# mathdiane/dNMF

Measured on AMD Instinct MI355X. Metric: frames/sec demixed, 512x512xT K=100, higher is better.
Workload: dtype f32

## Files before the change

### dnmf_amd/_lib.py

```python
from __future__ import annotations

import ctypes as C
import os

_HERE = os.path.dirname(os.path.abspath(__file__))
LIB_PATH = os.environ.get("DNMF_LIB") or os.path.join(_HERE, "libdnmf_hip.so")
ABI_VERSION = 6

_vp, _i, _l, _sz, _d = C.c_void_p, C.c_int, C.c_long, C.c_size_t, C.c_double

SIGNATURES = {
    "dnmf_version": (_i, []),
    "dnmf_last_error": (C.c_char_p, []),
    "dnmf_build_stamp": (C.c_char_p, []),
    "dnmf_padded_k": (_i, [_i]),
    "dnmf_pack_footprints": (_i, [_vp, _l, _i, _vp, _i, _vp]),
    "dnmf_warp_gather": (_i, [_vp, _i, _i, _i, _i, _vp, _i, _vp, _i, _vp, _vp, _vp]),
    "dnmf_halo_voxels": (_l, [_i, _i, _i]),
    "dnmf_halo_row": (_i, [_i, _i]),
    "dnmf_recon_image": (_i, [_vp, _i, _i, _i, _i, _i, _vp, _l, _vp, _i, _vp, _l, _vp]),
    "dnmf_warp_recon_grad_workspace": (_sz, [_i, _i, _i, _i]),
    "dnmf_warp_recon_grad": (_i, [_vp, _l, _vp, _vp, _l, _vp, _vp, _i, _i, _i, _vp, _i, _vp, _i, _i, _vp, _vp, _vp,
                                  _vp, _vp, _vp, _sz, _vp]),
    "dnmf_warp_gram_rhs_workspace": (_sz, [_l, _i, _i]),
    "dnmf_warp_gram_rhs": (_i, [_vp, _i, _i, _l, _i, _i, _i, _vp, _i, _vp, _i, _vp, _l, _vp, _vp, _vp, _vp, _sz,
                                _vp]),
    "dnmf_warp_gram_rhs_bf16": (_i, [_vp, _i, _i, _l, _i, _i, _i, _vp, _i, _vp, _i, _vp, _l, _vp, _vp, _vp, _vp, _sz,
                                     _vp]),
    "dnmf_sparse_k": (_i, [_i]),
    "dnmf_pack_footprints_sparse": (_i, [_vp, _l, _i, _vp, _vp, _i, _vp, _vp]),
    "dnmf_warp_gram_rhs_sparse_workspace": (_sz, [_l, _i, _i]),
    "dnmf_warp_gram_rhs_sparse": (_i, [_vp, _i, _i, _vp, _vp, _i, _i, _i, _vp, _i, _vp, _i, _vp, _l, _vp, _vp, _vp, _vp,
                                       _sz, _vp, _vp]),
    "dnmf_warp_gram_rhs_sparse_lt_workspace": (_sz, [_l, _i, _i]),
    "dnmf_warp_gram_rhs_sparse_lt": (_i, [_vp, _i, _i, _vp, _vp, _i, _i, _i, _vp, _i, _vp, _i, _vp, _l, _vp, _vp, _vp, _vp,
                                          _sz, _vp, _vp]),
    "dnmf_mu_temporal": (_i, [_vp, _vp, _vp, _l, _i, _i, _i, _vp]),
    "dnmf_mu_temporal_nbr": (_i, [_vp, _vp, _vp, _l, _i, _i, _i, _vp, _i, _vp]),
    "dnmf_mu_temporal_slots": (_i, [_vp, _i, _i, _vp, _vp, _l, _i, _i, _i, _vp, _i, _vp]),
    "dnmf_warp_gram_rhs_lists_chunks": (_i, [_i, _i, _i, _i]),
    "dnmf_mu_temporal_step": (_i, [_vp, _vp, _vp, _vp, _l, _i, _i, _d, _vp, _vp, _vp]),
    "dnmf_hals_temporal": (_i, [_vp, _vp, _vp, _l, _i, _i, _i, _vp, _i, _vp, _vp]),
    "dnmf_hals_temporal_slots": (_i, [_vp, _i, _i, _vp, _vp, _l, _i, _i, _i, _vp, _i, _vp, _vp]),
    "dnmf_hals_temporal_step": (_i, [_vp, _vp, _vp, _l, _i, _i, _d, _i, _vp, _i, _vp]),
    "dnmf_hals_temporal_kkt": (_i, [_vp, _vp, _vp, _l, _i, _i, _d, _vp, _i, _vp, _vp]),
    "dnmf_spatial_accum": (_i, [_vp, _l, _vp, _vp, _l, _vp, _l, _vp, _i, _l, _i, _vp, _vp, _i, _vp]),
    "dnmf_mu_spatial": (_i, [_vp, _vp, _vp, _vp, _d, _l, _i, _vp]),
    "dnmf_image_iwarp_workspace": (_sz, [_i, _i, _i, _i]),
    "dnmf_image_iwarp": (_i, [_vp, _l, _vp, _i, _i, _i, _vp, _i, _vp, _i, _vp, _l, _vp, _sz, _i, _vp, _vp]),
    "dnmf_image_iwarp_channels": (_i, [_vp, _l, _l, _i, _vp, _i, _i, _i, _vp, _i, _vp, _i, _vp, _l, _l, _vp, _sz, _i, _vp,
                                        _vp]),
    "dnmf_adam_epoch_workspace": (_sz, [_i]),
    "dnmf_adam_epoch": (_i, [_vp, _vp, _vp, _vp, _i, _l, _vp, _vp, _i, _d, _d, _d, _d, _i, _vp, _sz, _vp]),
    "dnmf_render_frames": (_i, [_vp, _vp, _i, _i, _i, _i, _i, _i, _i, _d, _d, _vp, _l, _vp]),
    "dnmf_lists_axis_masks_bytes": (_sz, [_i, _i, _i, _i]),
    "dnmf_pack_footprints_lists": (_i, [_vp, _i, _i, _i, _i, _vp, _vp, _vp, _vp, _vp, _vp]),
    "dnmf_warp_gram_rhs_lists_workspace": (_sz, [_i, _i, _i, _i, _i, _i]),
    "dnmf_warp_gram_rhs_lists": (_i, [_vp, _vp, _vp, _vp, _i, _i, _i, _i, _i, _vp, _i, _vp, _i, _vp, _l, _vp, _vp, _vp,
                                      _vp, _sz, _vp, _vp]),
    "dnmf_recon_image_lists": (_i, [_vp, _vp, _i, _i, _i, _i, _vp, _l, _vp, _i, _vp, _l, _vp]),
    "dnmf_recon_image_lists_ex": (_i, [_vp, _vp, _i, _i, _i, _i, _vp, _l, _vp, _i, _vp, _l, _i, _vp]),
    "dnmf_motion_grad_lists_workspace": (_sz, [_i, _i, _i, _i, _i]),
    "dnmf_motion_grad_lists": (_i, [_vp, _vp, _i, _vp, _l, _vp, _l, _vp, _i, _i, _i, _vp, _i, _vp, _i, _i, _vp, _vp, _vp, _i,
                                    _vp, _sz, _vp]),
    "dnmf_spatial_lists_tiles": (_l, [_i, _i, _i]),
    "dnmf_spatial_lists_setup": (_i, [_vp, _i, _i, _i, _i, _vp, _vp]),
    "dnmf_spatial_accum_lists_workspace": (_sz, [_i, _i, _i, _l, _i]),
    "dnmf_spatial_accum_lists": (_i, [_vp, _l, _vp, _vp, _l, _vp, _i, _i, _i, _i, _i, _vp, _l, _vp, _vp, _vp, _sz, _vp]),
    "dnmf_spatial_accum_lists_channels": (_i, [_vp, _l, _l, _i, _vp, _vp, _vp, _l, _vp, _i, _i, _i, _i, _i, _vp, _l, _vp, _vp,
                                                _vp, _sz, _vp]),
    "dnmf_mu_spatial_lists": (_i, [_vp, _vp, _vp, _vp, _vp, _d, _i, _i, _i, _i, _vp, _vp]),
    "dnmf_register_patches_grid": (_i, [_i, _i, _i, _vp, _vp, _vp, _vp]),
    "dnmf_register_patches_workspace": (_sz, [_i, _i, _i, _vp, _vp, _i]),
    "dnmf_register_patches": (_i, [_vp, _l, _vp, _i, _vp, _i, _i, _i, _vp, _vp, _vp, _i, _i, C.c_float, _vp, _vp, _vp, _sz, _vp]),
    "dnmf_rigid_correct_workspace": (_sz, [_i, _i, _i, _i]),
    "dnmf_rigid_correct": (_i, [_vp, _l, _vp, _i, _vp, _i, _i, _i, _vp, _i, C.c_float, _i, _vp, _vp, _l, _vp, _vp, _vp, _sz, _vp]),
    "dnmf_apply_pwrigid_workspace": (_sz, [_i, _i, _i, _vp, _vp, _i]),
    "dnmf_apply_pwrigid": (_i, [_vp, _l, _vp, _i, _i, _i, _i, _vp, _vp, _vp, C.c_float, _vp, _l, _vp, _vp, _vp, _sz, _vp]),
    "dnmf_apply_shifts_points": (_i, [_vp, _i, _vp, _i, _i, _vp, _vp, _vp]),
    "dnmf_nearest_points_workspace": (_sz, [_i, _i]),
    "dnmf_nearest_points": (_i, [_vp, _i, _l, _i, _vp, _l, _i, _i, _vp, _l, _vp, _l, _vp, _l, _vp, _sz, _vp]),
    "dnmf_fit_quadratic_warp": (_i, [_vp, _i, _i, _i, _vp, _i, _i, _i, _i, _d, _vp, _vp, _vp]),
    "dnmf_invert_quadratic_warp": (_i, [_vp, _i, _vp, _i, _vp, _i, _vp, _d, _vp, _vp]),
    "dnmf_roi_signals": (_i, [_vp, _l, _i, _i, _i, _vp, _i, _i, _i, _vp, _vp, _vp]),
    "dnmf_detect_neurons_workspace": (_sz, [_vp, _i, _d]),
    "dnmf_detect_neurons": (_i, [_vp, _vp, _i, _d, _d, _d, _d, _vp, _vp, _vp, _vp, _sz, _vp]),
    "dnmf_track_neurons": (_i, [_vp, _l, _vp, _i, _vp, _vp, _i, _i, _i, _d, _vp, _d, _vp, _vp, _vp, _vp, _vp]),
    "dnmf_warp_normal_eqs_workspace": (_sz, [_i, _i, _i, _i]),
    "dnmf_warp_normal_eqs": (_i, [_vp, _l, _vp, _vp, _l, _vp, _i, _i, _i, _vp, _i, _vp, _i, _vp, _vp, _vp, _i, _vp, _sz, _vp]),
    "dnmf_lm_step": (_i, [_vp, _vp, _vp, _i, _i, _vp, _vp, _i, _vp, _vp, _vp, _vp, _vp, _vp, _vp, _vp, _d, _d, _d, _d, _i, _vp]),
    "dnmf_lm_step_smooth": (_i, [_vp, _vp, _vp, _i, _i, _vp, _vp, _vp, _i, _vp, _vp, _vp, _vp, _vp, _vp, _vp, _vp, _d, _d, _d,
                                 _d, _i, _vp, _d, _vp, _vp]),
    "dnmf_warp_pullback": (_i, [_vp, _l, _l, _i, _vp, _i, _i, _i, _vp, _i, _vp, _i, _vp, _l, _l, _i, C.c_float, _vp, _vp, _vp]),
# ... 56 lines not shown
```

### dnmf_amd/csrc/warp_gram_lists.hip

```cpp
#include <cstdlib>

#include "warp_gram_lists.hpp"

namespace dnmf {

__global__ __launch_bounds__(256) void lists_axis_masks_kernel(const int *__restrict__ bbox, int K, Volume vol, int NW,
                                                               unsigned long long *__restrict__ masks) {
    const long e = (long)blockIdx.x * 256 + threadIdx.x;
    if (e >= axis_masks_entries(vol)) return;
    const int S[3] = {vol.X, vol.Y, vol.Z};
    long o = e;
    int d = 0;
    while (o >= 2L * (S[d] + 2)) o -= 2L * (S[d] + 2), ++d;
    const bool hi_table = o >= S[d] + 2;
    const int i = hi_table ? (int)(o - (S[d] + 2)) : (int)o - 1;
    for (int w = 0; w < NW; ++w) {
        unsigned long long m = 0;
        for (int j = 0; j < 64; ++j) {
            const int k = 64 * w + j;
            if (k >= K) break;
            const int lo = bbox[k * 6 + 2 * d], hi = bbox[k * 6 + 2 * d + 1];
            const bool in = lo <= hi && (hi_table ? hi >= i : lo <= i);
            m |= (unsigned long long)in << j;
        }
        masks[e * NW + w] = m;
    }
}

template <int NW>
__global__ __launch_bounds__(256) void lists_tilemask_kernel(ListParams p) {
    const long id = (long)blockIdx.x * 256 + threadIdx.x;
    if (id >= (long)p.B * p.ntiles) return;
    const int b = (int)(id / p.ntiles), q = (int)(id - (long)b * p.ntiles);
    const Volume vol = p.vol;
    const int t = p.times ? p.times[b] : b;
    float bt[30];
    load_beta(p.beta, p.T, t, bt);
    const int qx = q % p.ntx, rest = q / p.ntx, qz = rest % p.ntz, qy = rest / p.ntz;
    const int tx = LISTS_VPL << p.lgx, ty = 1 << p.lgy, tz = 1 << p.lgz;
    const int S[3] = {vol.X, vol.Y, vol.Z};
    const int first[3] = {qx * tx, qy * ty, qz * tz}, size[3] = {tx, ty, tz};
    float lo[3], hi[3];
#pragma unroll
    for (int d = 0; d < 3; ++d) lo[d] = (float)first[d], hi[d] = (float)min(first[d] + size[d] - 1, S[d] - 1);
    const bool hasz = vol.Z > 1;
    unsigned long long m[NW];
#pragma unroll
    for (int w = 0; w < NW; ++w) m[w] = ~0ull;
    int ta[3] = {0, 0, 0}, tc[3] = {0, 0, 0};
    bool finite = true;
#pragma unroll
    for (int d = 0; d < 3; ++d) {
        int a = 0, c = 0;
        if ((d < 2 || hasz) && !tap_range(bt, vol, d, lo, hi, hasz, a, c)) {
#pragma unroll
            for (int w = 0; w < NW; ++w) m[w] = 0;
            finite = false;
            continue;
        }
        ta[d] = a, tc[d] = c;
        const unsigned long long *LO = p.axis_masks + (axis_masks_offset(vol, d, 0) + (min(c, S[d]) + 1 < 0 ? 0 : min(c, S[d]) + 1)) * NW;
        const unsigned long long *HI = p.axis_masks + (axis_masks_offset(vol, d, 1) + min(max(a, 0), S[d] + 1)) * NW;
#pragma unroll
        for (int w = 0; w < NW; ++w) m[w] &= LO[w] & HI[w];
    }
#pragma unroll
    for (int w = 0; w < NW; ++w) p.tile_masks[id * NW + w] = m[w];
    int2 reg = make_int2(-1, 0);
    if (vol.Z <= 2 && finite && p.hl.Xp >= LISTS_RR && p.hl.rowf >= LISTS_RC && p.hl.Xp < 32768 && p.hl.rowf < 65536) {
        const int ax = max(ta[0], -HALO), cx = min(tc[0], vol.X + 1), ay = max(ta[1], -HALO), cy = min(tc[1], vol.Y + 1);
        const int r0 = min(ax + HALO, p.hl.Xp - LISTS_RR), c0 = min(((ay + HALO) * vol.Z) & ~3, p.hl.rowf - LISTS_RC);
        if (cx >= ax && cy >= ay && cx + HALO - r0 < LISTS_RR && (cy + HALO) * vol.Z + vol.Z - 1 - c0 < LISTS_RC)
            reg = make_int2(r0, c0);
    }
    int nlist = 0;
    unsigned ids = 0xffffffffu;
#pragma unroll
    for (int w = 0; w < NW; ++w) {
        unsigned long long rem = m[w];
        while (rem) {
            if (nlist < 4) ids = (ids & ~(0xffu << (8 * nlist))) | ((unsigned)(64 * w + __builtin_ctzll(rem)) << (8 * nlist));
            ++nlist, rem &= rem - 1;
        }
    }
    const int place = (qx < 65536 && rest < 32768) ? (qx | rest << 16) : -1;
    p.tile_desc[id] = make_int4(reg.x < 0 ? -1 : (reg.x << 16 | reg.y), (int)ids, nlist, place);
}

__global__ __launch_bounds__(256) void gram_lists_finish_kernel(const float *__restrict__ slab, int nchunks, int nslot,
                                                                const int *__restrict__ pair_slot, int K,
                                                                float *__restrict__ G, float *__restrict__ r) {
    const int b = blockIdx.x;
    const float *src = slab + (long)b * nchunks * nslot;
    for (int e = threadIdx.x; e < K * K + K; e += blockDim.x) {
        const int slot = e < K * K ? pair_slot[e] : e - K * K;
        float s = 0.0f;
        if (slot != nslot - 1)
            for (int c = 0; c < nchunks; ++c) s += src[(long)c * nslot + slot];
        if (e < K * K)
            G[(long)b * K * K + e] = s;
        else
            r[(long)b * K + (e - K * K)] = s;
    }
}

__global__ void lists_init_kernel(int *bbox, int K) {
    const int i = blockIdx.x * blockDim.x + threadIdx.x;
    if (i < K * 6) bbox[i] = (i & 1) ? -1 : 0x7fffffff;
}

__global__ __launch_bounds__(256) void lists_transpose_kernel(const float *__restrict__ A, long P, int K, Volume vol,
                                                              HaloLayout hl, float *__restrict__ At,
                                                              int *__restrict__ bbox) {
    __shared__ float tile[32][33];
    const long p0 = (long)blockIdx.x * 32;
    const int k0 = blockIdx.y * 32;
    const int tx = threadIdx.x & 31, ty = threadIdx.x >> 5;
    for (int i = ty; i < 32; i += 8) {
        const long pp = p0 + i;
        const int k = k0 + tx;
        tile[i][tx] = (pp < P && k < K) ? A[pp * K + k] : 0.0f;
    }
    __syncthreads();
    for (int i = ty; i < 32; i += 8) {
        const int k = k0 + i;
        const long pp = p0 + tx;
        const bool in = k < K && pp < P;
        const float v = in ? tile[tx][i] : 0.0f;
        int x = 0, y = 0, z = 0;
        if (in) {
            voxel_xyz(pp, vol, x, y, z);
            At[(long)k * hl.Pp + (long)(x + HALO) * hl.rowf + (long)(y + HALO) * vol.Z + z] = v;
        }
        const bool nz = v != 0.0f;
        const unsigned long long any = __ballot(nz);
        if (any == 0) continue;
        int lo[3] = {nz ? x : 0x7fffffff, nz ? y : 0x7fffffff, nz ? z : 0x7fffffff};
        int hi[3] = {nz ? x : -1, nz ? y : -1, nz ? z : -1};
#pragma unroll
// ... 46 lines not shown
        for (int l = k + 1; l < K; ++l) {
            const int v = meets(k, l) ? s++ : trash;
            pair_slot[k * K + l] = v;
            pair_slot[l * K + k] = v;
        }
    }
}

static void lists_tile_shape(const Volume &vol, int &lgx, int &lgy, int &lgz, int &ntx, int &nty, int &ntz, int &ntiles) {
    lgz = vol.Z == 1 ? 0 : (vol.Z == 2 ? 1 : 2);
    lgy = vol.Z == 1 ? 5 : 4;
    lgx = 6 - lgy - lgz;
    const int tx = LISTS_VPL << lgx, ty = 1 << lgy, tz = 1 << lgz;
    ntx = (vol.X + tx - 1) / tx;
    ntz = (vol.Z + tz - 1) / tz;
    nty = (vol.Y + ty - 1) / ty;
    ntiles = ntx * nty * ntz;
}

static long lists_max_chunks(int B) {
    const long want = (LISTS_ITEMS + B - 1) / B;
    return want < 1 ? 1 : (want > 64 ? 64 : want);
}

static void lists_choose_chunks(int ntiles, int B, int &nchunks, int &chunk_len) {
    long want = lists_max_chunks(B);
    if (const char *e = getenv("DNMF_LISTS_CHUNKS")) {
        const long n = strtol(e, nullptr, 10);
        if (n >= 1 && n <= want) want = n;
    }
    if (want > ntiles) want = ntiles;
    chunk_len = (int)((ntiles + want - 1) / want);
    nchunks = (ntiles + chunk_len - 1) / chunk_len;
}

static int lists_words(int K) { return K <= 64 ? 1 : (K <= 128 ? 2 : 4); }

static int lists_passes(int chunk_len) {
    if (const char *e = getenv("DNMF_LISTS_PASSES")) {
        if (e[0] == '1' && e[1] == 0) return 1;
        if (e[0] == '2' && e[1] == 0) return 2;
    }
    return chunk_len < 100 ? 1 : 2;
}

static void lists_plan(ListParams &p) {
    lists_tile_shape(p.vol, p.lgx, p.lgy, p.lgz, p.ntx, p.nty, p.ntz, p.ntiles);
    lists_choose_chunks(p.ntiles, p.B, p.nchunks, p.chunk_len);
    p.tables = p.nchunks * lists_passes(p.chunk_len);
}

template <int NW>
static void launch_tilemask(const ListParams &p, hipStream_t st) {
    const long nthreads = (long)p.B * p.ntiles;
    hipLaunchKernelGGL((lists_tilemask_kernel<NW>), dim3((unsigned)((nthreads + 255) / 256)), dim3(256), 0, st, p);
}

SideStream &side_stream() {
    static SideStream per_device[64];
    static std::mutex create;
    int dev = 0;
    if (hipGetDevice(&dev) != hipSuccess || dev < 0 || dev >= 64) dev = 0;
    SideStream &ss = per_device[dev];
    std::lock_guard<std::mutex> hold(create);
    if (!ss.stream) {
        hipStream_t s = nullptr;
        hipEvent_t a = nullptr, b = nullptr;
        if (hipStreamCreateWithFlags(&s, hipStreamNonBlocking) == hipSuccess &&
            hipEventCreateWithFlags(&a, hipEventDisableTiming) == hipSuccess &&
            hipEventCreateWithFlags(&b, hipEventDisableTiming) == hipSuccess)
            ss.stream = s, ss.fork = a, ss.join = b;
    }
    return ss;
}

}

extern "C" {

size_t dnmf_lists_axis_masks_bytes(int X, int Y, int Z, int K) {
    if (X <= 0 || Y <= 0 || Z <= 0 || K <= 0 || K > 64 * dnmf::LISTS_MAXW) return 0;
    return (size_t)dnmf::axis_masks_entries(dnmf::make_volume(X, Y, Z)) * dnmf::lists_words(K) * sizeof(unsigned long long);
}

int dnmf_pack_footprints_lists(const float *A, int X, int Y, int Z, int K, float *At, int *bbox, int *pair_slot,
                               int *nslot, void *axis_masks, dnmf_stream_t stream) {
    using namespace dnmf;
    DNMF_REQUIRE(A && At && bbox && pair_slot && nslot && axis_masks, DNMF_E_NULL, "dnmf_pack_footprints_lists: NULL buffer");
    DNMF_REQUIRE(X > 0 && Y > 0 && Z > 0 && K > 0, DNMF_E_SHAPE, "dnmf_pack_footprints_lists: X=%d Y=%d Z=%d K=%d", X, Y, Z,
                 K);
    DNMF_REQUIRE(K <= 64 * LISTS_MAXW, DNMF_E_UNSUPPORTED, "dnmf_pack_footprints_lists: K=%d > %d", K, 64 * LISTS_MAXW);
    const Volume vol = make_volume(X, Y, Z);
    const HaloLayout hl = make_halo_layout(X, Y, Z);
    hipStream_t st = (hipStream_t)stream;
    hipError_t e = hipMemsetAsync(At, 0, (size_t)K * hl.Pp * sizeof(float), st);
    DNMF_REQUIRE(e == hipSuccess, (int)e, "dnmf_pack_footprints_lists: hipMemsetAsync: %s", hipGetErrorString(e));
    hipLaunchKernelGGL(lists_init_kernel, dim3((K * 6 + 255) / 256), dim3(256), 0, st, bbox, K);
    hipLaunchKernelGGL(lists_transpose_kernel, dim3((unsigned)((vol.P + 31) / 32), (unsigned)((K + 31) / 32)), dim3(256), 0,
                       st, A, vol.P, K, vol, hl, At, bbox);
    hipLaunchKernelGGL(lists_pairs_kernel, dim3(1), dim3(256), 0, st, bbox, K, pair_slot, nslot);
    hipLaunchKernelGGL(lists_axis_masks_kernel, dim3((unsigned)((axis_masks_entries(vol) + 255) / 256)), dim3(256), 0, st, bbox,
                       K, vol, lists_words(K), static_cast<unsigned long long *>(axis_masks));
    return check_launch("dnmf_pack_footprints_lists");
}

static size_t lists_slab_bytes(int nslot, int B) {
    const size_t tables = 2 * (size_t)dnmf::lists_max_chunks(B);
    return ((size_t)B * tables * (size_t)nslot * sizeof(float) + 255) / 256 * 256;
}

static size_t lists_masks_bytes(int K, int B, int ntiles) {
    return ((size_t)B * ntiles * dnmf::lists_words(K) * sizeof(unsigned long long) + 15) / 16 * 16;
}

size_t dnmf_warp_gram_rhs_lists_workspace(int nslot, int K, int X, int Y, int Z, int B) {
    using namespace dnmf;
    if (nslot <= 0 || B <= 0 || K <= 0 || K > 64 * LISTS_MAXW || X <= 0 || Y <= 0 || Z <= 0) return 0;
    int lgx, lgy, lgz, ntx, nty, ntz, ntiles;
    lists_tile_shape(make_volume(X, Y, Z), lgx, lgy, lgz, ntx, nty, ntz, ntiles);
    return lists_slab_bytes(nslot, B) + lists_masks_bytes(K, B, ntiles) + (size_t)B * ntiles * sizeof(int4);
}

int dnmf_warp_gram_rhs_lists(const float *At, const int *bbox, const int *pair_slot, const void *axis_masks, int nslot, int K,
                             int X, int Y, int Z, const float *beta, int T, const int *times, int B, const float *frames,
                             long ldf, const int *frame_ids, float *G, float *r, void *workspace, size_t workspace_bytes,
                             unsigned long long *counters, dnmf_stream_t stream) {
    using namespace dnmf;
    DNMF_REQUIRE(At && bbox && pair_slot && axis_masks && beta && frames && workspace && (!G == !r), DNMF_E_NULL,
                 "dnmf_warp_gram_rhs_lists: NULL buffer");
    DNMF_REQUIRE(X > 0 && Y > 0 && Z > 0 && K > 0 && T > 0 && B > 0 && nslot > K, DNMF_E_SHAPE,
                 "dnmf_warp_gram_rhs_lists: X=%d Y=%d Z=%d K=%d T=%d B=%d nslot=%d", X, Y, Z, K, T, B, nslot);
    DNMF_REQUIRE(K <= 64 * LISTS_MAXW, DNMF_E_UNSUPPORTED, "dnmf_warp_gram_rhs_lists: K=%d > %d", K, 64 * LISTS_MAXW);
    DNMF_REQUIRE(nslot <= LISTS_MAX_SLOTS, DNMF_E_UNSUPPORTED,
                 "dnmf_warp_gram_rhs_lists: %d pattern slots > %d (footprints overlap too much for this kernel)", nslot,
                 LISTS_MAX_SLOTS);
    ListParams p;
    p.vol = make_volume(X, Y, Z);
    p.hl = make_halo_layout(X, Y, Z);
    DNMF_REQUIRE(ldf >= p.vol.P, DNMF_E_SHAPE, "dnmf_warp_gram_rhs_lists: ldf=%ld < P=%ld", ldf, p.vol.P);
    DNMF_REQUIRE(p.hl.Pp < (1L << 29) && p.hl.row4 < (1 << 23) && p.hl.Xp < (1 << 23), DNMF_E_UNSUPPORTED,
                 "dnmf_warp_gram_rhs_lists: volume %dx%dx%d too large for 32-bit tap offsets", X, Y, Z);
    p.At = At, p.bbox = bbox, p.pair_slot = pair_slot, p.nslot = nslot, p.K = K;
    p.axis_masks = static_cast<const unsigned long long *>(axis_masks);
    p.beta = beta, p.T = T, p.times = times, p.B = B;
    p.frames = frames, p.ldf = ldf, p.frame_ids = frame_ids;
    p.slab = static_cast<float *>(workspace);
    p.tile_masks = reinterpret_cast<unsigned long long *>(static_cast<char *>(workspace) + lists_slab_bytes(nslot, B));
    p.counters = counters;
    lists_plan(p);
    DNMF_REQUIRE(workspace_bytes >= dnmf_warp_gram_rhs_lists_workspace(nslot, K, X, Y, Z, B), DNMF_E_WORKSPACE,
                 "dnmf_warp_gram_rhs_lists: workspace %zu < %zu bytes", workspace_bytes,
                 dnmf_warp_gram_rhs_lists_workspace(nslot, K, X, Y, Z, B));
    hipStream_t st = (hipStream_t)stream;
    const long nitems = (long)p.nchunks * B;
    const unsigned nwg = (unsigned)((nitems + 3) / 4);
    const int nw = lists_words(K);
    p.tile_desc = reinterpret_cast<int4 *>(reinterpret_cast<char *>(p.tile_masks) + lists_masks_bytes(K, B, p.ntiles));
    const size_t lds = (((size_t)4 * nslot + 3) & ~(size_t)3) * sizeof(float) +
                       (Z <= 2 ? (size_t)4 * LISTS_NG * LISTS_REGION * sizeof(float) : 0);
    if (nw == 1) launch_tilemask<1>(p, st);
    else if (nw == 2) launch_tilemask<2>(p, st);
    else launch_tilemask<4>(p, st);
    if (Z > 1) {
        launch_lists_z(p, nwg, lds, st, nw);
    } else {
        if (nw == 1) launch_lists_t<1, 1>(p, nwg, lds, st);
        else if (nw == 2) launch_lists_t<1, 2>(p, nwg, lds, st);
        else launch_lists_t<1, 4>(p, nwg, lds, st);
    }
    if (G)
        hipLaunchKernelGGL(gram_lists_finish_kernel, dim3((unsigned)B), dim3(256), 0, st, p.slab, p.tables, nslot,
                           pair_slot, K, G, r);
    return check_launch("dnmf_warp_gram_rhs_lists");
}

int dnmf_warp_gram_rhs_lists_chunks(int X, int Y, int Z, int B) {
    using namespace dnmf;
    if (X <= 0 || Y <= 0 || Z <= 0 || B <= 0) return 0;
    ListParams p{};
    p.vol = make_volume(X, Y, Z), p.B = B;
    lists_plan(p);
    return p.tables;
}

}
```

### dnmf_amd/csrc/warp_gram_lists.hpp

```cpp
#pragma once
#include <mutex>
#include <type_traits>

#include "warp_taps.hpp"

namespace dnmf {

typedef float f32x4 __attribute__((ext_vector_type(4)));


constexpr int LISTS_WAVES = 4;
constexpr int LISTS_WAVES_Z2 = 4;
constexpr int LISTS_WAVES_Z2L = 3;
constexpr int LISTS_WAVES_Z3 = 3;

constexpr int LISTS_NG = 4;
constexpr int LISTS_LGV = 2;
constexpr int LISTS_VPL = 1 << LISTS_LGV;
constexpr int LISTS_MAXW = 4;
constexpr long LISTS_ITEMS = 16384;
constexpr int LISTS_MAX_SLOTS = 3800;
constexpr int LISTS_RR = 12, LISTS_RC = 40;
constexpr int LISTS_REGION = LISTS_RR * LISTS_RC;
static_assert(LISTS_RC % 4 == 0 && LISTS_REGION / 4 <= 128 && LISTS_REGION / 4 > 64, "stage_dma moves two pieces per lane");

struct ListParams {
    const float *At;
    const int *bbox;
    const int *pair_slot;
    const unsigned long long *axis_masks;
    int nslot;
    int K;
    Volume vol;
    HaloLayout hl;
    const float *beta;
    int T;
    const int *times;
    int B;
    const float *frames;
    long ldf;
    const int *frame_ids;
    float *slab;
    unsigned long long *tile_masks;
    int4 *tile_desc;
    int nchunks, chunk_len;
    int tables;
    int lgx, lgy, lgz;
    int ntx, nty, ntz, ntiles;
    unsigned long long *counters;
};

__host__ __device__ inline long axis_masks_offset(const Volume &vol, int d, int hi_table) {
    const int S[3] = {vol.X, vol.Y, vol.Z};
    long o = 0;
    for (int e = 0; e < d; ++e) o += 2L * (S[e] + 2);
    return o + (hi_table ? S[d] + 2 : 0);
}
__host__ __device__ inline long axis_masks_entries(const Volume &vol) { return 2L * (vol.X + vol.Y + vol.Z + 6); }

template <int ZM, int NW, int FAST, bool F32OFF, int PASS>
__global__ __launch_bounds__(256, (ZM == 1 ? LISTS_WAVES : (ZM == 2 ? (PASS == 2 ? LISTS_WAVES_Z2L : LISTS_WAVES_Z2) : LISTS_WAVES_Z3))) void warp_gram_lists_kernel(ListParams p) {
    constexpr bool LONGPASS = PASS == 2;
    extern __shared__ float s_tab[];
    constexpr bool HASZ = ZM > 1;
    constexpr int NPAIR = LISTS_NG * (LISTS_NG + 1) / 2;
    const int lane = threadIdx.x & 63;
    const int wave = __builtin_amdgcn_readfirstlane(threadIdx.x >> 6);
    const long item = (long)blockIdx.x * 4 + wave;
    if (item >= (long)p.nchunks * p.B) return;
    const int chunk = (int)(item / p.B);
    const int b = (int)(item - (long)chunk * p.B);
    const int t = p.times ? p.times[b] : b;
    const float *__restrict__ yb = p.frames + (long)(p.frame_ids ? p.frame_ids[b] : b) * p.ldf;
    const Volume vol = p.vol;
    const HaloLayout hl = p.hl;
    const int K = p.K;
    const size_t plane = (size_t)hl.Pp * 4u;

    float bt[30];
    load_beta(p.beta, p.T, t, bt);

    float *tab = s_tab + (size_t)wave * p.nslot;
    for (int i = lane; i < p.nslot; i += 64) tab[i] = 0.0f;
    const unsigned tab_lds = (unsigned)(size_t)(__attribute__((address_space(3))) float *)tab;
    char *stage_lds = reinterpret_cast<char *>(s_tab + (((size_t)4 * p.nslot + 3) & ~(size_t)3)) +
                      (size_t)wave * (LISTS_NG * LISTS_REGION * 4);
    constexpr int PPR = LISTS_RC / 4;
    const int piece_row[2] = {lane / PPR, (lane + 64) / PPR};
    const int piece_c4[2] = {lane - piece_row[0] * PPR, lane + 64 - piece_row[1] * PPR};
    const int4 *__restrict__ descs = p.tile_desc + (long)b * p.ntiles;

    const int lgx = p.lgx, lgz = p.lgz;
    const int lgy = p.lgy;
    const int lz = lane & ((1 << lgz) - 1), ly = (lane >> lgz) & ((1 << lgy) - 1), lx = lane >> (lgz + lgy);
    const int q_begin = chunk * p.chunk_len;
    const int q_end = min(q_begin + p.chunk_len, p.ntiles);
    const unsigned long long *__restrict__ masks = p.tile_masks + (long)b * p.ntiles * NW;
    unsigned long long n_eval = 0, n_pair = 0;
#ifdef DNMF_K3N_STAMPS
    unsigned long long st_acc[10] = {0, 0, 0, 0, 0, 0, 0, 0, 0, 0}, st_last = __builtin_amdgcn_s_memtime();
#define DNMF_STAMP(i)                                                     \
    {                                                                     \
        const unsigned long long now_ = __builtin_amdgcn_s_memtime();      \
        st_acc[i] += now_ - st_last, st_last = now_;                      \
    }
#else
#define DNMF_STAMP(i)
#endif

    __builtin_amdgcn_fence(__ATOMIC_RELEASE, "wavefront");
    __builtin_amdgcn_wave_barrier();
    __builtin_amdgcn_fence(__ATOMIC_ACQUIRE, "wavefront");

    auto add_slot = [&](int slot, float total_in_last_lane) {
        const unsigned addr = tab_lds + 4u * (unsigned)slot;
        if (lane == 63) asm volatile("ds_add_f32 %0, %1" : : "v"(addr), "v"(total_in_last_lane) : "memory");
    };
    auto pair_slot_of = [&](int k, int l) {
        return __builtin_amdgcn_readfirstlane(p.pair_slot[max(k, 0) * K + max(l, 0)]);
    };
    auto take_ids = [&](unsigned long long (&rem)[NW], int (&ks)[LISTS_NG]) {
#pragma unroll
        for (int i = 0; i < LISTS_NG; ++i) {
            int k = -1;
// ... 6 lines not shown
                found = found || take;
            }
            ks[i] = k;
        }
    };

    float acc_r[LISTS_NG], acc_p[NPAIR];
    int run_k[LISTS_NG];
    int run_n = 0;
    auto flush = [&]() {
        if (run_n == 0) return;
        auto go = [&](auto nn) {
            constexpr int N = decltype(nn)::value;
            int sl[N][N];
#pragma unroll
            for (int i = 0; i < N; ++i)
#pragma unroll
                for (int j = i; j < N; ++j) sl[i][j] = pair_slot_of(run_k[i], run_k[j]);
            float sr[N], sp[N][N];
            int e = 0;
#pragma unroll
            for (int i = 0; i < N; ++i) {
                sr[i] = wave_sum_last(acc_r[i]);
#pragma unroll
                for (int j = i; j < N; ++j) sp[i][j] = wave_sum_last(acc_p[e++]);
            }
#pragma unroll
            for (int i = 0; i < N; ++i) {
                add_slot(run_k[i], sr[i]);
#pragma unroll
                for (int j = i; j < N; ++j) add_slot(sl[i][j], sp[i][j]);
            }
        };
        using std::integral_constant;
        switch (run_n) {
            case 1: go(integral_constant<int, 1>{}); break;
            case 2: go(integral_constant<int, 2>{}); break;
            case 3: go(integral_constant<int, 3>{}); break;
            default: go(integral_constant<int, 4>{}); break;
        }
        static_assert(LISTS_NG == 4, "the dispatch above lists the group sizes");
        run_n = 0;
    };

    float b2[30];
    double_beta(bt, b2);
    Monomials<HASZ> mono = monomials<HASZ>(0.0f, 0.0f, 0.0f);
    int row_of_c = -1;
    unsigned long long prev[NW];
#pragma unroll
    for (int wd = 0; wd < NW; ++wd) prev[wd] = 0;
    int prev_ids = -1;

    for (int q0 = q_begin; q0 < q_end; q0 += 64) {
      unsigned my_lo[NW], my_hi[NW];
      int my_reg = -1;
      int my_ids = -1, my_n = 0;
      int my_place = -1;
      {
          const int ql = min(q0 + lane, q_end - 1);
          if (PASS != 1) {
#pragma unroll
              for (int wd = 0; wd < NW; ++wd) {
                  const unsigned long long m = masks[(long)ql * NW + wd];
                  my_lo[wd] = (unsigned)m, my_hi[wd] = (unsigned)(m >> 32);
              }
          }
          const int4 dsc = descs[ql];
          my_reg = ZM == 3 ? -1 : dsc.x, my_ids = dsc.y, my_n = dsc.z, my_place = dsc.w;
      }
      if (LONGPASS) {
          int myn = 0;
#pragma unroll
          for (int wd = 0; wd < NW; ++wd) myn += __builtin_popcount(my_lo[wd]) + __builtin_popcount(my_hi[wd]);
          if (__ballot(myn > LISTS_NG) == 0) continue;
      }
      const int q1 = min(q0 + 64, q_end);
      for (int q = q0; q < q1; ++q) {
        const int jl = q - q0;
        unsigned long long msk[NW];
        int n = 0;
        bool same = true;
        int ids = -1;
        if (PASS == 1) {
            n = __builtin_amdgcn_readlane(my_n, jl);
            if (n == 0 || n > LISTS_NG) continue;
            ids = __builtin_amdgcn_readlane(my_ids, jl);
            same = ids == prev_ids;
            prev_ids = ids;
        } else {
#pragma unroll
            for (int wd = 0; wd < NW; ++wd) {
                msk[wd] = ((unsigned long long)(unsigned)__builtin_amdgcn_readlane((int)my_hi[wd], jl) << 32) |
                          (unsigned)__builtin_amdgcn_readlane((int)my_lo[wd], jl);
                n += __builtin_popcountll(msk[wd]);
                same = same && msk[wd] == prev[wd];
            }
        }
        if (n == 0 || (PASS == 1 && n > LISTS_NG) || (PASS == 2 && n <= LISTS_NG)) continue;
        DNMF_STAMP(0)
#ifdef DNMF_K3N_STAMPS
        st_acc[7] += 1, st_acc[8] += n > LISTS_NG, st_acc[9] += (!same || n > LISTS_NG) && run_n != 0;
#endif
        if (!same || n > LISTS_NG) flush();
        DNMF_STAMP(1)
        if (PASS != 1) {
#pragma unroll
            for (int wd = 0; wd < NW; ++wd) prev[wd] = n > LISTS_NG ? 0 : msk[wd];
        }

        const int place = __builtin_amdgcn_readlane(my_place, jl);
        const int qx = place >= 0 ? (place & 0xffff) : q % p.ntx, rest = place >= 0 ? (place >> 16) : q / p.ntx;
        if (rest != row_of_c) {
            const int qz = HASZ ? rest % p.ntz : 0, qy = HASZ ? rest / p.ntz : rest;
            mono = monomials<HASZ>(0.0f, (float)((qy << lgy) + ly), (float)((qz << lgz) + lz));
            row_of_c = rest;
        }
        const int qz = HASZ ? rest % p.ntz : 0, qy = HASZ ? rest / p.ntz : rest;
        const int y = (qy << lgy) + ly, z = (qz << lgz) + lz;
        const bool yz_in = y < vol.Y && z < vol.Z;
        int reg_r0 = -1, reg_c0 = 0;
        if (ZM != 3) {
            const int rg = __builtin_amdgcn_readlane(my_reg, jl);
            reg_r0 = rg < 0 ? -1 : rg >> 16, reg_c0 = rg & 0xffff;
        }
        const bool staged = ZM != 3 && reg_r0 >= 0 && n <= (PASS == 2 ? 2 : 1) * LISTS_NG;
        const float lds_origin = 4.0f * (float)((HALO - reg_r0) * LISTS_RC + HALO * (ZM == 2 ? 2 : 1) - reg_c0);
        const unsigned reg_goff = (unsigned)(reg_r0 * hl.row4 + reg_c0 * 4);

        auto stage_load = [&](int k, f32x4 (&piece)[2]) {
            const char *__restrict__ Ak = reinterpret_cast<const char *>(p.At) + (size_t)k * plane + reg_goff;
#pragma unroll
            for (int j = 0; j < 2; ++j) {
                unsigned o = (unsigned)(piece_row[j] * hl.row4 + piece_c4[j] * 16);
                asm("" : "+v"(o));
                piece[j] = (j == 0 || lane + 64 < LISTS_REGION / 4) ? *reinterpret_cast<const f32x4 *>(Ak + o)
                                                                   : f32x4{0.f, 0.f, 0.f, 0.f};
            }
// ... 268 lines not shown
            }
            DNMF_STAMP(6)
            continue;
        }
        unsigned long long rem1[NW];
#pragma unroll
        for (int wd = 0; wd < NW; ++wd) rem1[wd] = msk[wd];
        for (int g1 = 0; g1 < n; g1 += LISTS_NG) {
            int kA[LISTS_NG];
            float aA[LISTS_NG][LISTS_VPL];
            take_ids(rem1, kA);
#pragma unroll
            for (int i = 0; i < LISTS_NG; ++i)
                if (kA[i] >= 0) {
                    eval(kA[i], aA[i]);
                } else {
#pragma unroll
                    for (int v = 0; v < LISTS_VPL; ++v) aA[i][v] = 0.0f;
                }
#pragma unroll
            for (int i = 0; i < LISTS_NG; ++i) {
                if (kA[i] < 0) continue;
                add_slot(kA[i], wave_sum_last(dot4(aA[i], yv, 0.0f)));
#pragma unroll
                for (int j = i; j < LISTS_NG; ++j)
                    if (kA[j] >= 0) add_slot(pair_slot_of(kA[i], kA[j]), wave_sum_last(dot4(aA[i], aA[j], 0.0f)));
            }
            unsigned long long rem2[NW];
#pragma unroll
            for (int wd = 0; wd < NW; ++wd) rem2[wd] = rem1[wd];
            for (int g2 = g1 + LISTS_NG; g2 < n; g2 += LISTS_NG) {
                int kB[LISTS_NG];
                take_ids(rem2, kB);
#pragma unroll
                for (int j = 0; j < LISTS_NG; ++j) {
                    if (kB[j] < 0) continue;
                    float aB[LISTS_VPL];
                    eval(kB[j], aB);
                    int sl[LISTS_NG];
#pragma unroll
                    for (int i = 0; i < LISTS_NG; ++i) sl[i] = pair_slot_of(kA[i], kB[j]);
                    float sp[LISTS_NG];
#pragma unroll
                    for (int i = 0; i < LISTS_NG; ++i) sp[i] = wave_sum_last(dot4(aA[i], aB, 0.0f));
#pragma unroll
                    for (int i = 0; i < LISTS_NG; ++i)
                        if (kA[i] >= 0) add_slot(sl[i], sp[i]);
                }
            }
        }
        DNMF_STAMP(6)
        }
      }
    }
    flush();

    __builtin_amdgcn_fence(__ATOMIC_RELEASE, "wavefront");
    __builtin_amdgcn_wave_barrier();
    __builtin_amdgcn_fence(__ATOMIC_ACQUIRE, "wavefront");
    float *out = p.slab + ((long)b * p.tables + (LONGPASS ? p.nchunks : 0) + chunk) * p.nslot;
    for (int i = lane; i < p.nslot; i += 64) out[i] = tab[i];
    if (p.counters && lane == 0) {
        atomicAdd(&p.counters[0], n_eval);
        atomicAdd(&p.counters[1], n_pair);
#ifdef DNMF_K3N_STAMPS
        DNMF_STAMP(5)
        for (int i = 0; i < 10; ++i) atomicAdd(&p.counters[2 + i], st_acc[i]);
#endif
    }
}
#undef DNMF_STAMP

struct SideStream {
    std::mutex lock;
    hipStream_t stream = nullptr;
    hipEvent_t fork = nullptr, join = nullptr;
};
SideStream &side_stream();

template <int ZM, int NW, int FAST, bool F32OFF>
void launch_lists_passes(const ListParams &p, unsigned nwg, size_t lds, hipStream_t st) {
    if (p.tables == p.nchunks) {
        hipLaunchKernelGGL((warp_gram_lists_kernel<ZM, NW, FAST, F32OFF, 0>), dim3(nwg), dim3(256), lds, st, p);
        return;
    }
    SideStream &ss = side_stream();
    std::lock_guard<std::mutex> hold(ss.lock);
    const bool forked = ss.stream && hipEventRecord(ss.fork, st) == hipSuccess &&
                        hipStreamWaitEvent(ss.stream, ss.fork, 0) == hipSuccess;
    if (forked) {
        hipLaunchKernelGGL((warp_gram_lists_kernel<ZM, NW, FAST, F32OFF, 2>), dim3(nwg), dim3(256), lds, ss.stream, p);
        const bool recorded = hipEventRecord(ss.join, ss.stream) == hipSuccess;
        hipLaunchKernelGGL((warp_gram_lists_kernel<ZM, NW, FAST, F32OFF, 1>), dim3(nwg), dim3(256), lds, st, p);
        if (!recorded || hipStreamWaitEvent(st, ss.join, 0) != hipSuccess)
            (void)hipStreamSynchronize(ss.stream);
    } else {
        hipLaunchKernelGGL((warp_gram_lists_kernel<ZM, NW, FAST, F32OFF, 1>), dim3(nwg), dim3(256), lds, st, p);
        hipLaunchKernelGGL((warp_gram_lists_kernel<ZM, NW, FAST, F32OFF, 2>), dim3(nwg), dim3(256), lds, st, p);
    }
}

template <int ZM, int NW>
void launch_lists_t(const ListParams &p, unsigned nwg, size_t lds, hipStream_t st) {
    if (p.vol.fastdiv && p.hl.f32off)
        launch_lists_passes<ZM, NW, 1, true>(p, nwg, lds, st);
    else if (p.vol.fastdiv)
// ... 9 lines not shown
```

### include/dnmf_hip.h

```cpp
#ifndef DNMF_HIP_H
#define DNMF_HIP_H

#include <stddef.h>

#ifdef __cplusplus
extern "C" {
#endif

#define DNMF_ABI_VERSION 6

#define DNMF_OK 0
#define DNMF_E_NULL (-1)
#define DNMF_E_SHAPE (-2)
#define DNMF_E_UNSUPPORTED (-3)
#define DNMF_E_WORKSPACE (-4)

typedef void *dnmf_stream_t;

#define DNMF_HALO 2
int dnmf_halo_row(int Y, int Z);
long dnmf_halo_voxels(int X, int Y, int Z);

int dnmf_version(void);
const char *dnmf_last_error(void);
const char *dnmf_build_stamp(void);

int dnmf_padded_k(int K);
int dnmf_pack_footprints(const float *A, long P, int K, float *Apk, int Kp, dnmf_stream_t stream);

int dnmf_warp_gather(const float *A, int X, int Y, int Z, int K, const float *beta, int T,
                     const int *times, int B, float *A_t, float *grid, dnmf_stream_t stream);

int dnmf_recon_image(const float *Apk, int X, int Y, int Z, int K, int Kp, const float *C, long ldc, const int *times,
                     int B, float *S, long lds, dnmf_stream_t stream);

size_t dnmf_warp_recon_grad_workspace(int X, int Y, int Z, int B);
int dnmf_warp_recon_grad(const float *S, long lds, const int *s_ids, const float *frames, long ldf,
                         const int *frame_ids, const float *gout, int X, int Y, int Z, const float *beta,
                         int T, const int *times, int B, int norm_frames, float *recon, float *grad, float *loss,
                         float *frame_loss, float *reg, void *workspace, size_t workspace_bytes,
                         dnmf_stream_t stream);

size_t dnmf_warp_gram_rhs_workspace(long P, int K, int B);
int dnmf_warp_gram_rhs(const float *Apk, int Kp, int K, long a_frame_stride, int X, int Y, int Z,
                       const float *beta, int T, const int *times, int B, const float *frames, long ldf,
                       const int *frame_ids, float *G, float *r, void *workspace, size_t workspace_bytes,
                       dnmf_stream_t stream);

int dnmf_warp_gram_rhs_bf16(const float *Apk, int Kp, int K, long a_frame_stride, int X, int Y, int Z,
                            const float *beta, int T, const int *times, int B, const float *frames, long ldf,
                            const int *frame_ids, float *G, float *r, void *workspace, size_t workspace_bytes,
                            dnmf_stream_t stream);

int dnmf_sparse_k(int K);
int dnmf_pack_footprints_sparse(const float *A, long P, int K, const int *order, float *Aps, int Ks,
                                unsigned char *row_mask, dnmf_stream_t stream);
size_t dnmf_warp_gram_rhs_sparse_workspace(long P, int K, int B);
int dnmf_warp_gram_rhs_sparse(const float *Aps, int Ks, int K, const int *order, const unsigned char *row_mask,
                              int X, int Y, int Z, const float *beta, int T, const int *times, int B,
                              const float *frames, long ldf, const int *frame_ids, float *G, float *r,
                              void *workspace, size_t workspace_bytes, unsigned long long *counters,
                              dnmf_stream_t stream);

size_t dnmf_warp_gram_rhs_sparse_lt_workspace(long P, int K, int B);
int dnmf_warp_gram_rhs_sparse_lt(const float *Aps, int Ks, int K, const int *order, const unsigned char *row_mask,
                                 int X, int Y, int Z, const float *beta, int T, const int *times, int B,
                                 const float *frames, long ldf, const int *frame_ids, float *G, float *r,
                                 void *workspace, size_t workspace_bytes, unsigned long long *counters,
                                 dnmf_stream_t stream);

size_t dnmf_lists_axis_masks_bytes(int X, int Y, int Z, int K);
int dnmf_pack_footprints_lists(const float *A, int X, int Y, int Z, int K, float *At, int *bbox, int *pair_slot,
                               int *nslot, void *axis_masks, dnmf_stream_t stream);
size_t dnmf_warp_gram_rhs_lists_workspace(int nslot, int K, int X, int Y, int Z, int B);
int dnmf_warp_gram_rhs_lists_chunks(int X, int Y, int Z, int B);
int dnmf_warp_gram_rhs_lists(const float *At, const int *bbox, const int *pair_slot, const void *axis_masks, int nslot,
                             int K, int X, int Y, int Z, const float *beta, int T, const int *times, int B,
                             const float *frames, long ldf, const int *frame_ids, float *G, float *r, void *workspace,
                             size_t workspace_bytes, unsigned long long *counters, dnmf_stream_t stream);

int dnmf_recon_image_lists(const float *At, const int *bbox, int K, int X, int Y, int Z, const float *C, long ldc,
                           const int *times, int B, float *S, long lds, dnmf_stream_t stream);
int dnmf_recon_image_lists_ex(const float *At, const int *bbox, int K, int X, int Y, int Z, const float *C, long ldc,
                              const int *times, int B, float *S, long lds, int skip_empty, dnmf_stream_t stream);

size_t dnmf_motion_grad_lists_workspace(int X, int Y, int Z, int chunk, int B);
int dnmf_motion_grad_lists(const float *At, const int *bbox, int K, const float *C, long ldc, const float *frames, long ldf,
                           const int *frame_ids, int X, int Y, int Z, const float *beta, int T, const int *times, int B,
                           int norm_frames, float *grad, float *frame_loss, float *reg, int chunk, void *workspace,
                           size_t workspace_bytes, dnmf_stream_t stream);

int dnmf_mu_temporal(const float *G, const float *r, float *C, long ldc, int K, int T, int iters,
                     dnmf_stream_t stream);
int dnmf_mu_temporal_nbr(const float *G, const float *r, float *C, long ldc, int K, int T, int iters, const int *nbr,
                         int NN, dnmf_stream_t stream);
int dnmf_mu_temporal_slots(const float *slab, int nchunks, int nslot, const int *pair_slot, float *C, long ldc, int K,
                           int T, int iters, const int *nbr, int NN, dnmf_stream_t stream);
int dnmf_mu_temporal_step(const float *G, const float *r, const double *Cin, double *Cout, long ldc, int K,
                          int T, double gamma, const double *c_left, const double *c_right,
                          dnmf_stream_t stream);

int dnmf_hals_temporal(const float *G, const float *r, float *C, long ldc, int K, int T, int iters, const int *nbr, int NN,
                       double *kkt, dnmf_stream_t stream);
int dnmf_hals_temporal_slots(const float *slab, int nchunks, int nslot, const int *pair_slot, float *C, long ldc, int K,
                             int T, int iters, const int *nbr, int NN, double *kkt, dnmf_stream_t stream);
int dnmf_hals_temporal_step(const float *G, const float *r, double *C, long ldc, int K, int T, double gamma, int parity,
                            const int *nbr, int NN, dnmf_stream_t stream);
int dnmf_hals_temporal_kkt(const float *G, const float *r, const double *C, long ldc, int K, int T, double gamma,
                           const int *nbr, int NN, double *kkt, dnmf_stream_t stream);

int dnmf_spatial_accum(const float *Y, long ldy, const int *frame_ids, const float *C, long ldc, const float *Ct,
                       long ldct, const int *times, int T, long P, int K, float *A1, float *Cs, int accumulate,
                       dnmf_stream_t stream);
int dnmf_mu_spatial(float *A, const float *A1, const float *Cs, const float *D, double gamma, long P, int K,
                    dnmf_stream_t stream);

#define DNMF_COMM_ID_BYTES 128
typedef void *dnmf_comm_t;
int dnmf_comm_unique_id(void *id_host);
int dnmf_comm_init(dnmf_comm_t *comm, const void *id_host, int nranks, int rank);
int dnmf_allreduce_sum_f32(dnmf_comm_t comm, float *buf, size_t count, dnmf_stream_t stream);
int dnmf_comm_destroy(dnmf_comm_t comm);

size_t dnmf_image_iwarp_workspace(int X, int Y, int Z, int B);
int dnmf_image_iwarp(const float *frames, long ldf, const int *frame_ids, int X, int Y, int Z, const float *beta,
                     int T, const int *times, int B, float *out, long ldo, void *workspace, size_t workspace_bytes,
                     int exhaustive, unsigned long long *fallback_count, dnmf_stream_t stream);
int dnmf_image_iwarp_channels(const float *frames, long ldf, long ldc_in, int nchan, const int *frame_ids, int X, int Y, int Z,
// ... 130 lines not shown
```

Measured before the change: 710,300.

## Compact long-list tile indices per chunk so the long pass skips short tiles

When the lists Gram/RHS runs in two passes, the tile-mask stage now runs one wavefront per (chunk, frame). It ballot-compacts the indices of tiles whose list exceeds LISTS_NG into the upper 16 bits of each descriptor's z field and zeroes the long-pass table when a chunk has none. The long pass then reads this compacted list, exits early for empty chunks, and walks only the long tiles instead of scanning every tile and ballot-skipping. The price is a less parallel mask kernel, since one wave now covers each chunk instead of one thread per tile. The first pass must mask n with 0xffff, and chunk length is capped at 65535 tiles.

```diff
diff --git a/dnmf_amd/_lib.py b/dnmf_amd/_lib.py
--- a/dnmf_amd/_lib.py
+++ b/dnmf_amd/_lib.py
@@ -39,6 +39,7 @@
     "dnmf_mu_temporal_nbr": (_i, [_vp, _vp, _vp, _l, _i, _i, _i, _vp, _i, _vp]),
     "dnmf_mu_temporal_slots": (_i, [_vp, _i, _i, _vp, _vp, _l, _i, _i, _i, _vp, _i, _vp]),
     "dnmf_warp_gram_rhs_lists_chunks": (_i, [_i, _i, _i, _i]),
+    "dnmf_warp_gram_rhs_lists_plan": (_i, [_i, _i, _i, _i, _i, _i, _vp]),
     "dnmf_mu_temporal_step": (_i, [_vp, _vp, _vp, _vp, _l, _i, _i, _d, _vp, _vp, _vp]),
     "dnmf_hals_temporal": (_i, [_vp, _vp, _vp, _l, _i, _i, _i, _vp, _i, _vp, _vp]),
     "dnmf_hals_temporal_slots": (_i, [_vp, _i, _i, _vp, _vp, _l, _i, _i, _i, _vp, _i, _vp, _vp]),
diff --git a/dnmf_amd/csrc/warp_gram_lists.hip b/dnmf_amd/csrc/warp_gram_lists.hip
--- a/dnmf_amd/csrc/warp_gram_lists.hip
+++ b/dnmf_amd/csrc/warp_gram_lists.hip
@@ -28,10 +28,8 @@
 }
 
 template <int NW>
-__global__ __launch_bounds__(256) void lists_tilemask_kernel(ListParams p) {
-    const long id = (long)blockIdx.x * 256 + threadIdx.x;
-    if (id >= (long)p.B * p.ntiles) return;
-    const int b = (int)(id / p.ntiles), q = (int)(id - (long)b * p.ntiles);
+__device__ inline int lists_tile_list(const ListParams &p, int b, int q) {
+    const long id = (long)b * p.ntiles + q;
     const Volume vol = p.vol;
     const int t = p.times ? p.times[b] : b;
     float bt[30];
@@ -85,6 +83,41 @@
     }
     const int place = (qx < 65536 && rest < 32768) ? (qx | rest << 16) : -1;
     p.tile_desc[id] = make_int4(reg.x < 0 ? -1 : (reg.x << 16 | reg.y), (int)ids, nlist, place);
+    return nlist;
+}
+
+template <int NW>
+__global__ __launch_bounds__(256) void lists_tilemask_kernel(ListParams p) {
+    const long id = (long)blockIdx.x * 256 + threadIdx.x;
+    if (id >= (long)p.B * p.ntiles) return;
+    const int b = (int)(id / p.ntiles);
+    lists_tile_list<NW>(p, b, (int)(id - (long)b * p.ntiles));
+}
+
+template <int NW>
+__global__ __launch_bounds__(256) void lists_tilemask_chunks_kernel(ListParams p) {
+    const int lane = threadIdx.x & 63;
+    const long item = (long)blockIdx.x * 4 + (threadIdx.x >> 6);
+    if (item >= (long)p.nchunks * p.B) return;
+    const int chunk = (int)(item / p.B), b = (int)(item - (long)chunk * p.B);
+    const int q_begin = chunk * p.chunk_len, q_end = min(q_begin + p.chunk_len, p.ntiles);
+    auto entry = [&](int e) { return reinterpret_cast<unsigned short *>(&p.tile_desc[(long)b * p.ntiles + q_begin + e].z) + 1; };
+    int count = 0;
+    for (int q0 = q_begin; q0 < q_end; q0 += 64) {
+        const int q = q0 + lane;
+        const bool is_long = q < q_end && lists_tile_list<NW>(p, b, q) > LISTS_NG;
+        const unsigned long long m = __ballot(is_long);
+        __builtin_amdgcn_fence(__ATOMIC_RELEASE, "wavefront");
+        __builtin_amdgcn_wave_barrier();
+        __builtin_amdgcn_fence(__ATOMIC_ACQUIRE, "wavefront");
+        if (is_long) *entry(count + __popcll(m & ((1ull << lane) - 1))) = (unsigned short)(q - q_begin);
+        count += __popcll(m);
+    }
+    if (lane == 0 && count < q_end - q_begin) *entry(count) = (unsigned short)LISTS_NO_TILE;
+    if (count == 0) {
+        float *table = p.slab + ((long)b * p.tables + p.nchunks + chunk) * p.nslot;
+        for (int i = lane; i < p.nslot; i += 64) table[i] = 0.0f;
+    }
 }
 
 __global__ __launch_bounds__(256) void gram_lists_finish_kernel(const float *__restrict__ slab, int nchunks, int nslot,
@@ -237,8 +270,13 @@
 
 template <int NW>
 static void launch_tilemask(const ListParams &p, hipStream_t st) {
-    const long nthreads = (long)p.B * p.ntiles;
-    hipLaunchKernelGGL((lists_tilemask_kernel<NW>), dim3((unsigned)((nthreads + 255) / 256)), dim3(256), 0, st, p);
+    if (p.tables == p.nchunks) {
+        const long nthreads = (long)p.B * p.ntiles;
+        hipLaunchKernelGGL((lists_tilemask_kernel<NW>), dim3((unsigned)((nthreads + 255) / 256)), dim3(256), 0, st, p);
+    } else {
+        const long nitems = (long)p.nchunks * p.B;
+        hipLaunchKernelGGL((lists_tilemask_chunks_kernel<NW>), dim3((unsigned)((nitems + 3) / 4)), dim3(256), 0, st, p);
+    }
 }
 
 SideStream &side_stream() {
@@ -341,6 +379,8 @@
     const unsigned nwg = (unsigned)((nitems + 3) / 4);
     const int nw = lists_words(K);
     p.tile_desc = reinterpret_cast<int4 *>(reinterpret_cast<char *>(p.tile_masks) + lists_masks_bytes(K, B, p.ntiles));
+    DNMF_REQUIRE(p.tables == p.nchunks || p.chunk_len <= (int)LISTS_NO_TILE, DNMF_E_UNSUPPORTED,
+                 "dnmf_warp_gram_rhs_lists: %d tiles per chunk > %u in two launches", p.chunk_len, LISTS_NO_TILE);
     const size_t lds = (((size_t)4 * nslot + 3) & ~(size_t)3) * sizeof(float) +
                        (Z <= 2 ? (size_t)4 * LISTS_NG * LISTS_REGION * sizeof(float) : 0);
     if (nw == 1) launch_tilemask<1>(p, st);
@@ -368,4 +408,18 @@
     return p.tables;
 }
 
-}
+int dnmf_warp_gram_rhs_lists_plan(int nslot, int K, int X, int Y, int Z, int B, long *plan) {
+    using namespace dnmf;
+    DNMF_REQUIRE(plan, DNMF_E_NULL, "dnmf_warp_gram_rhs_lists_plan: NULL buffer");
+    DNMF_REQUIRE(nslot > 0 && B > 0 && K > 0 && K <= 64 * LISTS_MAXW && X > 0 && Y > 0 && Z > 0, DNMF_E_SHAPE,
+                 "dnmf_warp_gram_rhs_lists_plan: X=%d Y=%d Z=%d K=%d B=%d nslot=%d", X, Y, Z, K, B, nslot);
+    ListParams p{};
+    p.vol = make_volume(X, Y, Z), p.B = B;
+    lists_plan(p);
+    const size_t masks = lists_slab_bytes(nslot, B), desc = masks + lists_masks_bytes(K, B, p.ntiles);
+    const long out[6] = {p.ntiles, p.nchunks, p.chunk_len, p.tables, (long)masks, (long)desc};
+    for (int i = 0; i < 6; ++i) plan[i] = out[i];
+    return 0;
+}
+
+}
diff --git a/dnmf_amd/csrc/warp_gram_lists.hpp b/dnmf_amd/csrc/warp_gram_lists.hpp
--- a/dnmf_amd/csrc/warp_gram_lists.hpp
+++ b/dnmf_amd/csrc/warp_gram_lists.hpp
@@ -19,6 +19,7 @@
 constexpr int LISTS_VPL = 1 << LISTS_LGV;
 constexpr int LISTS_MAXW = 4;
 constexpr long LISTS_ITEMS = 16384;
+constexpr unsigned LISTS_NO_TILE = 0xffffu;
 constexpr int LISTS_MAX_SLOTS = 3800;
 constexpr int LISTS_RR = 12, LISTS_RC = 40;
 constexpr int LISTS_REGION = LISTS_RR * LISTS_RC;
@@ -70,6 +71,10 @@
     if (item >= (long)p.nchunks * p.B) return;
     const int chunk = (int)(item / p.B);
     const int b = (int)(item - (long)chunk * p.B);
+    if constexpr (LONGPASS) {
+        const unsigned first = (unsigned)p.tile_desc[(long)b * p.ntiles + (long)chunk * p.chunk_len].z >> 16;
+        if (__builtin_amdgcn_readfirstlane(first) == LISTS_NO_TILE) return;
+    }
     const int t = p.times ? p.times[b] : b;
     const float *__restrict__ yb = p.frames + (long)(p.frame_ids ? p.frame_ids[b] : b) * p.ldf;
     const Volume vol = p.vol;
@@ -182,13 +187,22 @@
     for (int wd = 0; wd < NW; ++wd) prev[wd] = 0;
     int prev_ids = -1;
 
-    for (int q0 = q_begin; q0 < q_end; q0 += 64) {
+    const int walk_begin = LONGPASS ? 0 : q_begin, walk_end = LONGPASS ? q_end - q_begin : q_end;
+    for (int q0 = walk_begin; q0 < walk_end; q0 += 64) {
       unsigned my_lo[NW], my_hi[NW];
       int my_reg = -1;
       int my_ids = -1, my_n = 0;
       int my_place = -1;
+      int my_q = 0;
+      int batch = 64;
       {
-          const int ql = min(q0 + lane, q_end - 1);
+          int ql = min(q0 + lane, walk_end - 1);
+          if (LONGPASS) {
+              const unsigned entry = (unsigned)descs[q_begin + ql].z >> 16;
+              const unsigned long long over = __ballot(entry == LISTS_NO_TILE || q0 + lane >= walk_end);
+              batch = over ? __builtin_ctzll(over) : 64;
+              my_q = ql = q_begin + (entry == LISTS_NO_TILE ? 0 : (int)entry);
+          }
           if (PASS != 1) {
 #pragma unroll
               for (int wd = 0; wd < NW; ++wd) {
@@ -199,21 +213,16 @@
           const int4 dsc = descs[ql];
           my_reg = ZM == 3 ? -1 : dsc.x, my_ids = dsc.y, my_n = dsc.z, my_place = dsc.w;
       }
-      if (LONGPASS) {
-          int myn = 0;
-#pragma unroll
-          for (int wd = 0; wd < NW; ++wd) myn += __builtin_popcount(my_lo[wd]) + __builtin_popcount(my_hi[wd]);
-          if (__ballot(myn > LISTS_NG) == 0) continue;
-      }
-      const int q1 = min(q0 + 64, q_end);
-      for (int q = q0; q < q1; ++q) {
-        const int jl = q - q0;
+      const int q1 = LONGPASS ? q0 + batch : min(q0 + 64, q_end);
+      for (int qi = q0; qi < q1; ++qi) {
+        const int jl = qi - q0;
+        const int q = LONGPASS ? __builtin_amdgcn_readlane(my_q, jl) : qi;
         unsigned long long msk[NW];
         int n = 0;
         bool same = true;
         int ids = -1;
         if (PASS == 1) {
-            n = __builtin_amdgcn_readlane(my_n, jl);
+            n = __builtin_amdgcn_readlane(my_n, jl) & 0xffff;
             if (n == 0 || n > LISTS_NG) continue;
             ids = __builtin_amdgcn_readlane(my_ids, jl);
             same = ids == prev_ids;
@@ -588,6 +597,7 @@
         DNMF_STAMP(6)
         }
       }
+      if (LONGPASS && batch < 64) break;
     }
     flush();
 
diff --git a/include/dnmf_hip.h b/include/dnmf_hip.h
--- a/include/dnmf_hip.h
+++ b/include/dnmf_hip.h
@@ -74,6 +74,7 @@
                                int *nslot, void *axis_masks, dnmf_stream_t stream);
 size_t dnmf_warp_gram_rhs_lists_workspace(int nslot, int K, int X, int Y, int Z, int B);
 int dnmf_warp_gram_rhs_lists_chunks(int X, int Y, int Z, int B);
+int dnmf_warp_gram_rhs_lists_plan(int nslot, int K, int X, int Y, int Z, int B, long *plan);
 int dnmf_warp_gram_rhs_lists(const float *At, const int *bbox, const int *pair_slot, const void *axis_masks, int nslot,
                              int K, int X, int Y, int Z, const float *beta, int T, const int *times, int B,
                              const float *frames, long ldf, const int *frame_ids, float *G, float *r, void *workspace,
```

Result: slower. 700,400 (-1.4%).
